# linnanwang/FastGen

Measured on AMD Instinct MI355X. Metric: images/sec at 4-step distilled (DMD2) sampling, higher is better.
Workload: dtype fp32 (tensors, accumulate) with split-bf16 x3 MFMA conv products; 1 GPU; EDM CIFAR-10 32x32 SongUNet (55.7M params) DMD2 4-step 'sde' sampling, batch=512 per GPU; global_batch=512, sample_steps=4, parallelism=replicas x1 (no data-path collective), graph=True

## Files before the change

### fastgen_amd/_lib.py

```python
import ctypes
import os
from ctypes import POINTER, c_char_p, c_double, c_float, c_int, c_int64, c_size_t, c_uint64, c_void_p

_HERE = os.path.dirname(os.path.abspath(__file__))
LIB_PATH = os.path.join(_HERE, "libfastgen_amd.so")

FG_MAX_LEVELS = 8
FG_DTYPE_F32, FG_DTYPE_BF16, FG_DTYPE_BF16X3 = 0, 1, 2
DTYPE_NAMES = {"fp32": FG_DTYPE_F32, "bf16": FG_DTYPE_BF16, "bf16x3": FG_DTYPE_BF16X3}
FG_SAMPLE_SDE, FG_SAMPLE_ODE = 0, 1
SAMPLE_TYPES = {"sde": FG_SAMPLE_SDE, "ode": FG_SAMPLE_ODE}
FG_LOOP_X0, FG_LOOP_MEANFLOW, FG_LOOP_EULER = 0, 1, 2
LOOP_KINDS = {"x0": FG_LOOP_X0, "meanflow": FG_LOOP_MEANFLOW, "euler": FG_LOOP_EULER}
FG_SCHEDULE_EDM, FG_SCHEDULE_RF = 0, 1
FG_DROP_PRECOND_INPUT, FG_DROP_PRECOND_OUTPUT = 1, 2
FG_BWD_DECODER, FG_BWD_ENCODER, FG_BWD_EMBED = 1, 2, 4
FG_MODEL_SONGUNET, FG_MODEL_DHARIWAL = 0, 1


class fg_edm_config(ctypes.Structure):
    _fields_ = [
        ("img_resolution", c_int), ("img_channels", c_int), ("label_dim", c_int), ("augment_dim", c_int),
        ("model_channels", c_int), ("num_levels", c_int), ("channel_mult", c_int * FG_MAX_LEVELS),
        ("channel_mult_emb", c_int), ("num_blocks", c_int), ("num_attn_resolutions", c_int),
# ... 44 lines not shown
    "fg_edm_destroy": (None, [c_void_p]),
    "fg_edm_num_params": (c_int, [c_void_p]),
    "fg_edm_param_info": (c_int, [c_void_p, c_int, POINTER(c_char_p), POINTER(c_int), POINTER(c_int64)]),
    "fg_edm_bind_param": (c_int, [c_void_p, c_char_p, c_void_p, c_int64]),
    "fg_edm_pack_weights": (c_int, [c_void_p, c_void_p]),
    "fg_edm_workspace_bytes": (c_size_t, [c_void_p, c_int]),
    "fg_edm_forward": (c_int, [c_void_p, c_void_p, c_void_p, c_void_p, c_void_p, c_void_p, c_void_p, c_int, c_void_p,
                               c_size_t, c_void_p]),
    "fg_edm_num_feature_taps": (c_int, [c_void_p]),
    "fg_edm_feature_info": (c_int, [c_void_p, c_int, POINTER(c_char_p), POINTER(c_int), POINTER(c_int)]),
    "fg_edm_forward_features": (c_int, [c_void_p, c_void_p, c_void_p, c_void_p, c_void_p, c_void_p, POINTER(c_void_p), c_int,
                                        c_void_p, c_size_t, c_void_p]),
    "fg_sampler_run": (c_int, [c_void_p, c_void_p, c_void_p, POINTER(c_double), c_int, c_int, c_int, c_void_p, c_uint64,
                               c_void_p, c_int, c_void_p, c_size_t, c_int, c_void_p]),
    "fg_edm_t_list": (c_int, [c_int, POINTER(c_double)]),
    "fg_rf_t_list": (c_int, [c_int, POINTER(c_double)]),
    "fg_edm_profile_begin": (c_int, [c_void_p]),
    "fg_edm_profile_end": (c_int, [c_void_p, POINTER(c_int64), POINTER(c_double), POINTER(c_double)]),
    "fg_edm_num_blocks": (c_int, [c_void_p]),
    "fg_edm_block_info": (c_int, [c_void_p, c_int, POINTER(c_char_p), POINTER(c_int), POINTER(c_int), POINTER(c_int),
                                  POINTER(c_int), POINTER(c_int)]),
    "fg_edm_run_block": (c_int, [c_void_p, c_int, c_void_p, c_int, c_void_p, c_int, c_void_p, c_void_p, c_int, c_void_p,
                                 c_size_t, c_void_p]),
    "fg_op_gn_coeffs": (c_int, [c_void_p, c_int, c_void_p, c_int, c_void_p, c_void_p, c_float, c_void_p, c_int, c_int, c_void_p]),
    "fg_op_adm_conv_pack_bytes": (c_size_t, [c_int, c_int, c_int, c_int]),
    "fg_op_adm_conv_pack": (c_int, [c_int, c_void_p, c_void_p, c_int, c_int, c_int, c_void_p]),
    "fg_op_adm_conv": (c_int, [c_int, c_int, c_void_p, c_int, c_void_p, c_int, c_int, c_int, c_int, c_int, c_void_p, c_int, c_void_p,
                               c_void_p, c_void_p, c_int, c_void_p, c_int, c_void_p]),
    "fg_op_adm_gn_workspace_bytes": (c_size_t, [c_int, c_int, c_int]),
    "fg_op_adm_gn_coeffs": (c_int, [c_void_p, c_int, c_void_p, c_int, c_void_p, c_void_p, c_float, c_void_p, c_int, c_void_p, c_int,
                                    c_int, c_void_p, c_size_t, c_void_p]),
    "fg_op_adm_attention": (c_int, [c_void_p, c_void_p, c_int, c_int, c_int, c_void_p]),
    "fg_op_adm_map_in": (c_int, [c_void_p, c_void_p, c_void_p, c_void_p, c_int, c_void_p, c_int, c_int, c_void_p]),
    "fg_op_latents": (c_int, [c_void_p, c_double, c_void_p, c_int64, c_void_p]),
    "fg_op_forward_process": (c_int, [c_void_p, c_void_p, c_double, c_int, c_void_p, c_int64, c_void_p]),
    "fg_op_x0_to_eps": (c_int, [c_void_p, c_void_p, c_double, c_int, c_void_p, c_int64, c_void_p]),
    "fg_op_conv_wgrad_workspace_bytes": (ctypes.c_size_t, [c_int, c_int, c_int, c_int, c_int]),
    "fg_op_conv_wgrad": (c_int, [c_void_p, c_void_p, c_void_p, c_int, c_int, c_int, c_int, c_int, c_int, c_void_p, ctypes.c_size_t, c_void_p]),
    "fg_op_conv_wgrad_f32": (c_int, [c_void_p, c_void_p, c_void_p, c_int, c_int, c_int, c_int, c_int, c_int, c_void_p, ctypes.c_size_t, c_void_p]),
    "fg_edm_bind_grad": (c_int, [c_void_p, c_char_p, c_void_p, c_int64]),
    "fg_edm_block_backward_workspace_bytes": (c_size_t, [c_void_p, c_int, c_int]),
    "fg_edm_run_block_backward": (c_int, [c_void_p, c_int, c_void_p, c_int, c_void_p, c_int, c_void_p, c_void_p, c_void_p,
                                          c_void_p, c_void_p, c_int, c_void_p, c_size_t, c_void_p]),
    "fg_edm_backward_workspace_bytes": (c_size_t, [c_void_p, c_int]),
    "fg_edm_backward": (c_int, [c_void_p, c_void_p, c_void_p, c_void_p, c_void_p, c_void_p, c_void_p, c_int, c_int, c_void_p,
                                c_size_t, c_void_p]),
# ... 101 lines not shown
```

### fastgen_amd/csrc/conv.h

```cpp
#pragma once
#include <hip/hip_runtime.h>

struct ConvArgs {
    const void* src1;
    const void* src2;
    int C1, C2;
    int Hs, Ws;
    int H, W;
    int B;
    const float2* ab;
    const void* wpack;
    const void* wpack_ws;
    const float* bias;
    const float* temb;
    int temb_stride;
    const void* resid;
    int rshift = 0;
    float scale;
    void* out;
    int Cout;
    float2* stats;
    int dbg;
    void* q_out;
    void* k_out;
// ... 2 lines not shown
    int gate_stride = 0;
    int act = 0;
    int heads = 0, head_dim = 0;
    size_t heads_lo_off = 0;
};

enum { PRO_NONE = 0, PRO_GN = 1, PRO_GN_SILU = 2 };
enum { RES_NONE = 0, RES_DOWN = 1, RES_UP = 2, RES_SUBPIX = 3 };
enum { OUT_NHWC = 0, OUT_QKV = 1, OUT_TOK = 2, OUT_HEADS = 3 };

int launch_conv_fused(int dtype, int ks, int pro, int res, int outmode, const ConvArgs& a, hipStream_t stream);
int conv_stat_slots(int W);
bool conv_ws_supported(int dtype, int ks, int pro, int res, int outmode, const ConvArgs& a);
bool conv_ws_enabled();
int launch_conv_ws(int res, const ConvArgs& a, hipStream_t stream, bool prepare_only, int pro = PRO_GN_SILU);
bool conv_ws_shape_ok(int dtype, int cout, int cin, int res);
int launch_pack_conv_weights_ws(const float* w_oihw, void* wpack_ws, int cout, int cin, hipStream_t stream);
bool conv_x3ws_supported(int ks, int pro, int res, int outmode, const ConvArgs& a);
bool conv_x3ws_shape_ok(int cout, int cin, int res);
int conv_x3ws_stat_slots(int W, int res);
int launch_conv_x3ws(int res, const ConvArgs& a, hipStream_t stream, bool prepare_only, int pro = PRO_GN_SILU);
int launch_pack_conv_weights_x3ws(const float* w_oihw, void* wpack_ws, int cout, int cin, hipStream_t stream);
int launch_pack_conv_weights_x3sub(const float* w_oihw, void* wpack_sub, int cout, int cin, hipStream_t stream);
int conv_subpix_mode();
int conv_launch_stat_slots(int dtype, int ks, int pro, int res, int outmode, const ConvArgs& a);
int launch_conv_ws_debug(const ConvArgs& a, int abl, hipStream_t stream);
int launch_conv_debug(int dtype, const ConvArgs& a, hipStream_t stream);
int conv_prepare_all(int dtype);
size_t conv_pack_elems(int cout, int cin, int ks);
int launch_pack_conv_weights(int dtype, const float* w_oihw, void* wpack, int cout, int cin, int ks, int qkv_perm,
                             hipStream_t stream);
```

### fastgen_amd/csrc/conv.hip

```cpp
#include "common.h"
#include "conv.h"
#include <stdlib.h>
#include <string.h>

#include <type_traits>

namespace {

constexpr int PITCH = 144;
constexpr int NTHR = 256;

template <int KS, int LOGW>
struct Geom {
    static constexpr int W = 1 << LOGW;
    static constexpr int LOGTW = (LOGW == 5) ? 4 : LOGW;
    static constexpr int TW = 1 << LOGTW;
    static constexpr int LOGTH = 3;
    static constexpr int TH = 1 << LOGTH;
    static constexpr int IMGS = 128 / (TH * TW);
    static constexpr int TCOLS = W / TW;
    static constexpr int TPI = (IMGS > 1) ? 1 : (W / TH) * TCOLS;
    static constexpr int PAD = KS / 2;
    static constexpr int HW_ = TW + 2 * PAD;
    static constexpr int HH_ = TH + 2 * PAD;
// ... 558 lines not shown
        case 4: return launch_one<__bf16, 3, PRO_GN_SILU, RES_NONE, 5, OUT_NHWC, 4>(a, stream);
        case 5: return launch_one<__bf16, 3, PRO_GN_SILU, RES_NONE, 5, OUT_NHWC, 5>(a, stream);
        case 6: return launch_one<__bf16, 3, PRO_GN_SILU, RES_NONE, 5, OUT_NHWC, 6>(a, stream);
        case 7: return launch_one<__bf16, 3, PRO_GN_SILU, RES_NONE, 5, OUT_NHWC, 7>(a, stream);
    }
    return (int)hipErrorInvalidValue;
}

int launch_conv_fused(int dtype, int ks, int pro, int res, int outmode, const ConvArgs& a, hipStream_t stream) {
    const int kc = dtype == 1 ? DT<__bf16>::KC : DT<float>::KC;
    if (a.H != a.W || (a.W != 8 && a.W != 16 && a.W != 32)) return (int)hipErrorInvalidValue;
    const bool tok = outmode == OUT_TOK || outmode == OUT_HEADS;
    if ((a.C1 % kc) || (a.C2 % kc) || (a.Cout % (tok ? 64 : 256)) || a.B <= 0) return (int)hipErrorInvalidValue;
    if (outmode == OUT_HEADS && (a.heads <= 0 || (a.head_dim % 4) || a.Cout != 3 * a.heads * a.head_dim || ((a.heads * a.head_dim) % 64) ||
                                 !a.q_out || !a.k_out || !a.vt_out))
        return (int)hipErrorInvalidValue;
    if (res == RES_NONE && (a.Hs != a.H || a.Ws != a.W)) return (int)hipErrorInvalidValue;
    if (res == RES_DOWN && (a.Hs != 2 * a.H || a.Ws != 2 * a.W)) return (int)hipErrorInvalidValue;
    if ((res == RES_UP || res == RES_SUBPIX) && (2 * a.Hs != a.H || 2 * a.Ws != a.W)) return (int)hipErrorInvalidValue;
    if (pro != PRO_NONE && !a.ab) return (int)hipErrorInvalidValue;
    if (outmode == OUT_QKV && (a.Cout != 768 || a.W > 16)) return (int)hipErrorInvalidValue;
    if (conv_ws_enabled() && conv_ws_supported(dtype, ks, pro, res, outmode, a)) return launch_conv_ws(res, a, stream, false, pro);
    if (dtype == 2 && conv_ws_enabled() && conv_x3ws_supported(ks, pro, res, outmode, a)) return launch_conv_x3ws(res, a, stream, false, pro);
    if (res == RES_SUBPIX || a.rshift) return (int)hipErrorInvalidValue;
    return dispatch_t(dtype, ks, pro, res, outmode, a, stream);
}

bool conv_ws_enabled() {
    static const bool on = [] {
        const char* e = getenv("FASTGEN_AMD_CONV_WS");
        return !(e && e[0] == '0');
    }();
    return on;
}

int conv_subpix_mode() {
    static const int mode = [] {
        const char* e = getenv("FASTGEN_AMD_CONV_SUBPIX");
        if (e && e[0] == '0') return 0;
        return (e && !strcmp(e, "skip")) ? 1 : 2;
    }();
    return mode;
}

int conv_launch_stat_slots(int dtype, int ks, int pro, int res, int outmode, const ConvArgs& a) {
    if (dtype == 2 && conv_ws_enabled() && conv_x3ws_supported(ks, pro, res, outmode, a)) return conv_x3ws_stat_slots(a.W, res);
// ... 16 lines not shown
                rc = dispatch_t(dtype, 3, PRO_GN_SILU, res, OUT_NHWC, a, nullptr);
            if (!rc) rc = dispatch_t(dtype, 1, PRO_NONE, res, OUT_NHWC, a, nullptr);
        }
        if (!rc) rc = dispatch_t(dtype, 3, PRO_NONE, RES_NONE, OUT_NHWC, a, nullptr);
        if (!rc && a.W <= 16) rc = dispatch_t(dtype, 1, PRO_GN, RES_NONE, OUT_QKV, a, nullptr);
        if (!rc && a.W == 16) rc = dispatch_t(dtype, 1, PRO_NONE, RES_NONE, OUT_TOK, a, nullptr);
        if (!rc && a.W == 16) rc = dispatch_t(dtype, 1, PRO_NONE, RES_NONE, OUT_HEADS, a, nullptr);
    }
    g_prepare_only = false;
    if (!rc && dtype == 2) {
        ConvArgs w{};
        for (int res : {RES_NONE, RES_UP})
            for (int ww : {32, 16, 8}) {
                if (ww == 8 && res != RES_NONE) continue;
                w.W = w.H = ww;
                if (!rc) rc = launch_conv_x3ws(res, w, nullptr, true, PRO_GN_SILU);
                if (!rc && res == RES_NONE) rc = launch_conv_x3ws(res, w, nullptr, true, PRO_NONE);
            }
        for (int ws_ : {16, 8}) {
            w.Ws = w.Hs = ws_;
            w.W = w.H = 2 * ws_;
            if (!rc) rc = launch_conv_x3ws(RES_SUBPIX, w, nullptr, true, PRO_GN_SILU);
        }
    }
    if (!rc && dtype == 1) {
        ConvArgs w{};
        for (int res : {RES_NONE, RES_UP}) {
            w.W = w.H = 32;
            if (!rc) rc = launch_conv_ws(res, w, nullptr, true);
            if (res == RES_NONE) {
                w.C1 = -128;
                if (!rc) rc = launch_conv_ws(res, w, nullptr, true);
                w.C1 = 0;
            }
            w.W = w.H = 16;
            if (!rc) rc = launch_conv_ws(res, w, nullptr, true);
        }
    }
    return rc;
}

size_t conv_pack_elems(int cout, int cin, int ks) { return (size_t)cout * cin * ks * ks; }

int launch_pack_conv_weights(int dtype, const float* w, void* out, int cout, int cin, int ks, int qkv_perm,
                             hipStream_t stream) {
    const size_t total = conv_pack_elems(cout, cin, ks);
// ... 10 lines not shown
```

### fastgen_amd/csrc/engine.hip

```cpp
#include <hip/hip_runtime.h>

#include <cmath>
#include <cstdarg>
#include <cstdio>
#include <cstdlib>
#include <cstring>
#include <string>
#include <map>
#include <vector>

#include "../../include/fastgen_amd.h"
#include "common.h"
#include "adm.h"
#include "edm2.h"
#include "conv.h"
#include "misc.h"

namespace {

thread_local std::string g_err;

int fail(int code, const char* fmt, ...) {
    char buf[512];
    va_list ap;
// ... 12 lines not shown

struct Param {
    std::string name;
    int ndim = 0;
    int64_t shape[4] = {1, 1, 1, 1};
    int64_t numel = 0;
    const float* ptr = nullptr;
    float* grad = nullptr;
};

enum Kind { K_STEM, K_BLOCK, K_AUX_NORM, K_AUX_CONV };

struct Block {
    std::string key;
    Kind kind = K_BLOCK;
    int cin = 0, cout = 0, res_in = 0, res_out = 0;
    bool up = false, down = false, attn = false, has_skip = false, is_dec = false;
    int skip_c = 0;
    int temb_off = 0;
    int norm0_w = -1, norm0_b = -1, conv0_w = -1, conv0_b = -1, aff_w = -1, aff_b = -1, norm1_w = -1, norm1_b = -1,
        conv1_w = -1, conv1_b = -1, skip_w = -1, skip_b = -1, norm2_w = -1, norm2_b = -1, qkv_w = -1, qkv_b = -1,
        proj_w = -1, proj_b = -1, w = -1, b = -1;
    void *p_conv0 = nullptr, *p_conv1 = nullptr, *p_skip = nullptr, *p_qkv = nullptr, *p_proj = nullptr;
    void *p_conv0_ws = nullptr, *p_conv1_ws = nullptr;
    void* p_conv0_sub = nullptr;
    int tap = -1;
    float* qkv_bias = nullptr;
    void* p_aux = nullptr;
    void* p_stem = nullptr;
};

struct Arena {
    char* base = nullptr;
    size_t off = 0, cap = 0;
    bool dry = false;
    void* take(size_t bytes) {
        off = (off + 255) & ~(size_t)255;
        void* p = dry ? nullptr : base + off;
        off += bytes;
        return p;
    }
    template <typename T>
    T* get(size_t n) {
        return reinterpret_cast<T*>(take(n * sizeof(T)));
    }
};
// ... 623 lines not shown
        HIP_TRY(launch_gn_finalize(x1.st, c1, x1.slots, c2 ? x2.st : nullptr, c2, c2 ? x2.slots : 0, gamma, beta, kBlockEps, ab, B, hw, s, mr));
    else
        HIP_TRY(launch_gn_coeffs(dtype, x1.p, c1, c2 ? x2.p : nullptr, c2, gamma, beta, kBlockEps, ab, B, hw, s, mr));
    return FG_OK;
}

void use_stash(Workspace& w, const BlockStash& st) {
    w.h.p = st.h;
    w.ab0 = st.ab0, w.ab1 = st.ab1, w.mr0 = st.mr0, w.mr1 = st.mr1;
    w.a1d = st.a1d;
    w.drop.block = st.index;
    if (st.xattn) {
        w.xattn.p = st.xattn;
        w.ab2 = st.ab2, w.mr2 = st.mr2;
        w.q = st.q, w.k = st.k, w.vt = st.vt, w.aout = st.aout;
    }
}
int block_index(const fg_edm* h, const Block* b) {
    for (size_t i = 0; i < h->blocks.size(); ++i)
        if (h->blocks[i] == b) return (int)i;
    return -1;
}

int run_block(fg_edm* h, const Block& b, const Act& x1, int c1, const Act& x2, int c2, const float* temb, Act& out, int B,
              Workspace& w, hipStream_t s) {
    if (c1 + c2 != b.cin) return fail(FG_EINVAL, "%s: got %d+%d input channels, expected %d", b.key.c_str(), c1, c2, b.cin);
    const int hw_in = b.res_in * b.res_in, hw = b.res_out * b.res_out;
    const int res_mode = b.down ? RES_DOWN : (b.up ? RES_UP : RES_NONE);
    const int slots = conv_stat_slots(b.res_out);
    int rc;
    if ((rc = norm_coeffs(h->dtype, x1, c1, x2, c2, h->P(b.norm0_w), h->P(b.norm0_b), w.ab0, B, hw_in, s, w.mr0))) return rc;
    ConvArgs a{};
    a.src1 = x1.p; a.src2 = c2 ? x2.p : nullptr; a.C1 = c1; a.C2 = c2;
    a.Hs = a.Ws = b.res_in; a.H = a.W = b.res_out; a.B = B;
    a.ab = w.ab0; a.wpack = b.p_conv0; a.wpack_ws = b.p_conv0_ws; a.bias = h->P(b.conv0_b);
    a.temb = temb + b.temb_off; a.temb_stride = h->temb_total;
    a.resid = nullptr; a.scale = 1.0f; a.out = w.h.p; a.Cout = b.cout; a.stats = w.h.st;
    const bool x3_up = b.up && w.infer && !w.a1d && h->cmode == FG_DTYPE_BF16X3 && conv_ws_enabled();
    bool sub0 = false;
    if (x3_up && conv_subpix_mode() == 2 && b.p_conv0_sub) {
        ConvArgs p = a;
        p.wpack_ws = b.p_conv0_sub;
        sub0 = conv_x3ws_supported(3, PRO_GN_SILU, RES_SUBPIX, OUT_NHWC, p);
    }
    if (sub0) {
        a.wpack_ws = b.p_conv0_sub;
// ... 22 lines not shown
        }
        ConvArgs k{};
        k.src1 = x1.p; k.src2 = c2 ? x2.p : nullptr; k.C1 = c1; k.C2 = c2;
        k.Hs = k.Ws = b.res_in; k.H = k.W = low ? b.res_in : b.res_out; k.B = B;
        k.wpack = b.p_skip; k.bias = h->P(b.skip_b); k.scale = 1.0f; k.out = w.sbuf; k.Cout = b.cout;
        HIP_TRY(conv_launch(h, 1, PRO_NONE, low ? RES_NONE : res_mode, OUT_NHWC, k, s));
        resid = w.sbuf;
        d.rshift = low ? 1 : 0;
    }
    HIP_TRY(launch_gn_finalize(w.h.st, b.cout, w.h.slots, nullptr, 0, 0, h->P(b.norm1_w), h->P(b.norm1_b), kBlockEps, w.ab1, B, hw, s, w.mr1));
    Act& x_mid = b.attn ? w.xattn : out;
    d.resid = resid; d.out = x_mid.p; d.stats = x_mid.st;
    if (w.a1d) {
        HIP_TRY(launch_gn_act(h->dtype, 0, w.h.p, b.cout, nullptr, 0, w.ab1, w.a1d, B, b.res_out, 0, s, w.drop));
        d.src1 = w.a1d; d.ab = nullptr;
        x_mid.slots = conv_launch_stat_slots(h->cmode, 3, PRO_NONE, RES_NONE, OUT_NHWC, d);
        HIP_TRY(conv_launch(h, 3, PRO_NONE, RES_NONE, OUT_NHWC, d, s));
    } else {
        x_mid.slots = conv_launch_stat_slots(h->cmode, 3, PRO_GN_SILU, RES_NONE, OUT_NHWC, d);
        HIP_TRY(conv_launch(h, 3, PRO_GN_SILU, RES_NONE, OUT_NHWC, d, s));
    }
    if (b.attn) {
        HIP_TRY(launch_gn_finalize(x_mid.st, b.cout, x_mid.slots, nullptr, 0, 0, h->P(b.norm2_w), h->P(b.norm2_b), kBlockEps, w.ab2, B, hw, s, w.mr2));
        ConvArgs q{};
        q.src1 = x_mid.p; q.C1 = b.cout; q.Hs = q.Ws = q.H = q.W = b.res_out; q.B = B;
        q.ab = w.ab2; q.wpack = b.p_qkv; q.bias = b.qkv_bias; q.scale = 1.0f; q.Cout = 3 * b.cout;
        q.q_out = w.q; q.k_out = w.k; q.vt_out = w.vt;
        HIP_TRY(conv_launch(h, 1, PRO_GN, RES_NONE, OUT_QKV, q, s));
        HIP_TRY(launch_attention(h->cmode, w.q, w.k, w.vt, w.aout, B, hw, s));
        ConvArgs p{};
        p.src1 = w.aout; p.C1 = b.cout; p.Hs = p.Ws = p.H = p.W = b.res_out; p.B = B;
        p.wpack = b.p_proj; p.bias = h->P(b.proj_b); p.resid = x_mid.p; p.scale = kSkipScale; p.out = out.p; p.Cout = b.cout;
        p.stats = out.st;
        HIP_TRY(conv_launch(h, 1, PRO_NONE, RES_NONE, OUT_NHWC, p, s));
        out.slots = slots;
    }
    return FG_OK;
}

int run_mapping(fg_edm* h, const float* labels, int B, Workspace& w, hipStream_t s) {
    const fg_edm_config& c = h->cfg;
    HIP_TRY(launch_mapping_in(w.coef + B, w.coef + 4 * (size_t)B, h->freqs, labels, c.label_dim,
                              h->P(h->find("model.map_label.weight")), h->P(h->find("model.map_label.bias")), w.emb0, B,
                              h->cond_ch, h->noise_ch, s, h->augment, h->augment ? h->P(h->find("model.map_augment.weight")) : nullptr, c.augment_dim));
    HIP_TRY(launch_linear(w.emb0, h->P(h->find("model.map_layer0.weight")), h->P(h->find("model.map_layer0.bias")), w.emb1,
                          B, h->cond_ch, h->emb_ch, 1, s));
    HIP_TRY(launch_linear(w.emb1, h->P(h->find("model.map_layer1.weight")), h->P(h->find("model.map_layer1.bias")), w.emb, B,
                          h->emb_ch, h->emb_ch, 1, s));
    HIP_TRY(launch_linear(w.emb, h->aff_w, h->aff_b, w.temb, B, h->emb_ch, h->temb_total, 0, s));
    return FG_OK;
}

int run_forward(fg_edm* h, const float* x_t, const double* t, int t_stride, const double* r, int r_stride,
                const float* labels, float* out, int B, Workspace& w, hipStream_t s, float* const* feats = nullptr,
                bool early = false, TrainStash* ts = nullptr) {
    if (h->adm) return adm_forward(h, x_t, t, t_stride, labels, out, B, w, s);
// ... 68 lines not shown
}

int ensure_device_state(fg_edm* h) {
    if (h->device_ready) return FG_OK;
    int rc;
    const size_t tsz = h->dtype ? 2 : 4;
    for (Block* b : h->blocks) {
        if ((rc = h->alloc(&b->p_conv0, conv_pack_elems(b->cout, b->cin, 3) * tsz))) return rc;
        if ((rc = h->alloc(&b->p_conv1, conv_pack_elems(b->cout, b->cout, 3) * tsz))) return rc;
        const bool x3 = h->cmode == FG_DTYPE_BF16X3;
        if ((x3 ? conv_x3ws_shape_ok(b->cout, b->cin, b->res_out) : conv_ws_shape_ok(h->cmode, b->cout, b->cin, b->res_out)) && !b->down &&
            (rc = h->alloc(&b->p_conv0_ws, conv_pack_elems(b->cout, b->cin, 3) * tsz)))
            return rc;
        if ((x3 ? conv_x3ws_shape_ok(b->cout, b->cout, b->res_out) : conv_ws_shape_ok(h->cmode, b->cout, b->cout, b->res_out)) &&
            (rc = h->alloc(&b->p_conv1_ws, conv_pack_elems(b->cout, b->cout, 3) * tsz)))
            return rc;
        if (x3 && b->up && conv_x3ws_shape_ok(b->cout, b->cin, b->res_in) && (rc = h->alloc(&b->p_conv0_sub, conv_pack_elems(b->cout, b->cin, 4) * 4)))
            return rc;
        if (b->has_skip && (rc = h->alloc(&b->p_skip, conv_pack_elems(b->cout, b->cin, 1) * tsz))) return rc;
        if (b->attn) {
            if ((rc = h->alloc(&b->p_qkv, conv_pack_elems(3 * b->cout, b->cout, 1) * tsz))) return rc;
            if ((rc = h->alloc(&b->p_proj, conv_pack_elems(b->cout, b->cout, 1) * tsz))) return rc;
            if ((rc = h->alloc((void**)&b->qkv_bias, sizeof(float) * 3 * b->cout))) return rc;
        }
    }
    for (Block& b : h->enc)
        if (b.kind == K_STEM && stem_supported(b.res_out, b.cin, b.cout))
            if ((rc = h->alloc(&b.p_stem, stem_pack_elems() * tsz))) return rc;
    for (Block& b : h->dec)
        if (b.kind == K_AUX_CONV && aux_head_supported(h->cmode, b.res_out, b.cin, b.cout))
            if ((rc = h->alloc(&b.p_aux, aux_pack_elems(b.cin) * tsz))) return rc;
    if ((rc = h->alloc((void**)&h->aff_w, sizeof(float) * (size_t)h->temb_total * h->emb_ch))) return rc;
    if ((rc = h->alloc((void**)&h->aff_b, sizeof(float) * (size_t)h->temb_total))) return rc;
    const int half = h->noise_ch / 2;
    std::vector<float> fr(half);
    for (int j = 0; j < half; ++j) fr[j] = powf(1.0f / 10000.0f, (float)j / (float)(half - 1));
    if ((rc = h->alloc((void**)&h->freqs, sizeof(float) * half))) return rc;
    HIP_TRY(hipMemcpy(h->freqs, fr.data(), sizeof(float) * half, hipMemcpyHostToDevice));
    if (conv_prepare_all(h->cmode) != 0) return fail(FG_EHIP, "hipFuncSetAttribute(dynamic LDS) failed");
    if (launch_attention(h->cmode, nullptr, nullptr, nullptr, nullptr, 1, 256, nullptr) != 0) return fail(FG_EHIP, "attention prepare failed");
    h->device_ready = true;
    return FG_OK;
}

#include "engine_adm.inc"

// ... 80 lines not shown
        ++h->pack_epoch;
        if ((rc = adm_pack_weights(h, s))) return rc;
        h->sampler.graph.drop();
        h->packed = true;
        return FG_OK;
    }
    if ((rc = ensure_device_state(h)) || (rc = h->check_bound(unused))) return rc;
    ++h->pack_epoch;
    for (Block* b : h->blocks) {
        HIP_TRY(launch_pack_conv_weights(h->cmode, h->P(b->conv0_w), b->p_conv0, b->cout, b->cin, 3, 0, s));
        HIP_TRY(launch_pack_conv_weights(h->cmode, h->P(b->conv1_w), b->p_conv1, b->cout, b->cout, 3, 0, s));
        if (h->cmode == FG_DTYPE_BF16X3) {
            if (b->p_conv0_ws) HIP_TRY(launch_pack_conv_weights_x3ws(h->P(b->conv0_w), b->p_conv0_ws, b->cout, b->cin, s));
            if (b->p_conv0_sub) HIP_TRY(launch_pack_conv_weights_x3sub(h->P(b->conv0_w), b->p_conv0_sub, b->cout, b->cin, s));
            if (b->p_conv1_ws) HIP_TRY(launch_pack_conv_weights_x3ws(h->P(b->conv1_w), b->p_conv1_ws, b->cout, b->cout, s));
        } else {
            if (b->p_conv0_ws) HIP_TRY(launch_pack_conv_weights_ws(h->P(b->conv0_w), b->p_conv0_ws, b->cout, b->cin, s));
            if (b->p_conv1_ws) HIP_TRY(launch_pack_conv_weights_ws(h->P(b->conv1_w), b->p_conv1_ws, b->cout, b->cout, s));
        }
        if (b->has_skip) HIP_TRY(launch_pack_conv_weights(h->cmode, h->P(b->skip_w), b->p_skip, b->cout, b->cin, 1, 0, s));
        if (b->attn) {
            HIP_TRY(launch_pack_conv_weights(h->cmode, h->P(b->qkv_w), b->p_qkv, 3 * b->cout, b->cout, 1, 1, s));
            HIP_TRY(launch_pack_conv_weights(h->cmode, h->P(b->proj_w), b->p_proj, b->cout, b->cout, 1, 0, s));
            for (int plane = 0; plane < 3; ++plane)
                HIP_TRY(hipMemcpy2DAsync(b->qkv_bias + plane * b->cout, sizeof(float), h->P(b->qkv_b) + plane,
                                         3 * sizeof(float), sizeof(float), b->cout, hipMemcpyDeviceToDevice, s));
        }
        HIP_TRY(hipMemcpyAsync(h->aff_w + (size_t)b->temb_off * h->emb_ch, h->P(b->aff_w),
                               sizeof(float) * (size_t)b->cout * h->emb_ch, hipMemcpyDeviceToDevice, s));
        HIP_TRY(hipMemcpyAsync(h->aff_b + b->temb_off, h->P(b->aff_b), sizeof(float) * b->cout, hipMemcpyDeviceToDevice, s));
    }
    for (Block& b : h->enc)
        if (b.kind == K_STEM && b.p_stem) HIP_TRY(launch_pack_stem_weights(h->dtype, h->P(b.w), b.p_stem, b.cin, s));
    for (Block& b : h->dec)
        if (b.kind == K_AUX_CONV && b.p_aux) HIP_TRY(launch_pack_aux_weights(h->cmode, h->P(b.w), b.p_aux, b.cin, b.cout, s));
    h->sampler.graph.drop();
    h->packed = true;
    return FG_OK;
}

size_t fg_edm_workspace_bytes(const fg_edm* h, int batch) {
    if (!h || batch <= 0) return 0;
    Arena A;
    A.dry = true;
    Workspace w;
    return plan_workspace(h, batch, A, w);
// ... 142 lines not shown
    HIP_TRY(hipMalloc(&wp, (size_t)256 * cin * ks * ks * 4));
    {
        const size_t blk = 4u << 20;
        std::vector<uint16_t> hb(blk / 2);
        uint32_t st = 0x12345u;
        for (auto& v : hb) {
            st = st * 1664525u + 1013904223u;
            v = (uint16_t)(((st >> 16) & 0x8000u) | ((0x78u + ((st >> 12) & 7u)) << 7) | ((st >> 20) & 0x7fu));
        }
        auto fill = [&](void* dst, size_t bytes) -> int {
            for (size_t o = 0; o < bytes; o += blk)
                HIP_TRY(hipMemcpy((char*)dst + o, hb.data(), std::min(blk, bytes - o), hipMemcpyHostToDevice));
            return FG_OK;
        };
        int rc;
        if ((rc = fill(x, npix * cin * 4)) || (rc = fill(resid, npix * 256 * 4)) || (rc = fill(ab, (size_t)batch * cin * 8)) ||
            (rc = fill(wp, (size_t)256 * cin * ks * ks * (dtype == 1 ? 2 : 4))))
            return rc;
    }
    HIP_TRY(hipMemset(bias, 0, 256 * 4));
    if (conv_prepare_all(dtype) != 0) return fail(FG_EHIP, "prepare failed");
    ConvArgs a{};
    a.src1 = x; a.C1 = cin; a.Hs = a.Ws = a.H = a.W = res; a.B = batch;
    a.ab = ab; a.wpack = wp; a.wpack_ws = wp; a.bias = bias; a.resid = with_resid ? resid : nullptr; a.scale = 1.f; a.out = out; a.Cout = 256;
    a.dbg = dbg;
    hipEvent_t e0, e1;
    HIP_TRY(hipEventCreate(&e0));
    HIP_TRY(hipEventCreate(&e1));
    auto run = [&]() { return dbg >= 64 ? launch_conv_ws_debug(a, dbg - 64, nullptr) : dbg < 0 ? launch_conv_fused(dtype, ks, ks == 3 ? PRO_GN_SILU : PRO_NONE, RES_NONE, OUT_NHWC, a, nullptr) : launch_conv_debug(dtype, a, nullptr); };
    for (int i = 0; i < 3; ++i) HIP_TRY(run());
    HIP_TRY(hipEventRecord(e0, nullptr));
    for (int i = 0; i < iters; ++i) HIP_TRY(run());
    HIP_TRY(hipEventRecord(e1, nullptr));
    HIP_TRY(hipEventSynchronize(e1));
    float ms = 0.f;
    HIP_TRY(hipEventElapsedTime(&ms, e0, e1));
    if (ms_out) *ms_out = ms / iters;
    (void)hipEventDestroy(e0); (void)hipEventDestroy(e1);
    (void)hipFree(x); (void)hipFree(out); (void)hipFree(resid); (void)hipFree(bias); (void)hipFree(ab); (void)hipFree(wp);
    return FG_OK;
}

int fg_edm_num_blocks(const fg_edm* h) {
    if (h && h->adm) return adm_num_blocks(h);
    return h ? (int)h->blocks.size() : 0;
}

// ... 15 lines not shown
                     int batch, void* workspace, size_t workspace_bytes, void* stream) {
    if (!h || !x1 || !emb || !out) return fail(FG_EINVAL, "null argument");
    if (h->adm) return adm_run_block(h, index, x1, c1, x2, c2, emb, out, batch, workspace, workspace_bytes, (hipStream_t)stream);
    if (!h->packed) return fail(FG_ENOTREADY, "weights are not packed (call fg_edm_pack_weights)");
    if (index < 0 || index >= (int)h->blocks.size()) return fail(FG_EINVAL, "block index out of range");
    Workspace w;
    int rc0 = setup_ws(plan_workspace, h, batch, workspace, workspace_bytes, w);
    if (rc0) return rc0;
    hipStream_t s = (hipStream_t)stream;
    HIP_TRY(launch_linear(emb, h->aff_w, h->aff_b, w.temb, batch, h->emb_ch, h->temb_total, 0, s));
    const Block& b = *h->blocks[index];
    const size_t npix_in = (size_t)batch * b.res_in * b.res_in, npix_out = (size_t)batch * b.res_out * b.res_out;
    Act a1, a2;
    HIP_TRY(launch_to_act(h->dtype, x1, w.cvt1, (int64_t)npix_in * c1, s));
    a1.p = w.cvt1;
    if (c2) {
        HIP_TRY(launch_to_act(h->dtype, x2, w.cvt2, (int64_t)npix_in * c2, s));
        a2.p = w.cvt2;
    }
    w.infer = true;
    int rc = run_block(h, b, a1, c1, a2, c2, w.temb, w.xa, batch, w, s);
    if (rc) return rc;
    HIP_TRY(launch_from_act(h->dtype, w.xa.p, out, (int64_t)npix_out * b.cout, s));
    return FG_OK;
}

#include "engine_train.inc"
#include "engine_dit.inc"
#include "engine_wan.inc"
#include "engine_sampler.inc"
#include "engine_edm2.inc"

int fg_op_gn_coeffs(const float* x1, int c1, const float* x2, int c2, const float* gamma, const float* beta, float eps,
                    float* ab_out, int batch, int hw, void* stream) {
    if (!x1 || !gamma || !beta || !ab_out) return fail(FG_EINVAL, "null argument");
    HIP_TRY(launch_gn_coeffs(0, x1, c1, c2 ? x2 : nullptr, c2, gamma, beta, eps, (float2*)ab_out, batch, hw, (hipStream_t)stream));
    return FG_OK;
}

size_t fg_op_adm_conv_pack_bytes(int mode, int cout, int cin, int ks) {
    if ((mode != FG_DTYPE_BF16 && mode != FG_DTYPE_BF16X3) || (ks != 1 && ks != 3) || cout <= 0 || cin <= 0 || cin % 32) return 0;
    return adm_conv_pack_elems(mode, cout, cin, ks) * sizeof(__bf16);
}
int fg_op_adm_conv_pack(int mode, const float* w_oihw, void* packed, int cout, int cin, int ks, void* stream) {
    if (!fg_op_adm_conv_pack_bytes(mode, cout, cin, ks))
        return fail(FG_EINVAL, "fg_op_adm_conv_pack: mode %d (1 bf16, 2 bf16x3), ks %d (1, 3), cout %d > 0, cin %d (multiple of 32)", mode,
// ... 270 lines not shown
```

### include/fastgen_amd.h

```cpp
#ifndef FASTGEN_AMD_H
#define FASTGEN_AMD_H

#include <stddef.h>
#include <stdint.h>

#ifdef __cplusplus
extern "C" {
#endif

#define FG_API __attribute__((visibility("default")))

#define FG_OK 0
#define FG_EINVAL 1
#define FG_ENOTREADY 2
#define FG_EHIP 3
#define FG_ENOMEM 4

#define FG_DTYPE_F32 0
#define FG_DTYPE_BF16 1
#define FG_DTYPE_BF16X3 2

#define FG_SAMPLE_SDE 0
#define FG_SAMPLE_ODE 1

// ... 55 lines not shown

FG_API int fg_edm_num_feature_taps(const fg_edm* h);
FG_API int fg_edm_feature_info(const fg_edm* h, int index, const char** key, int* channels, int* resolution);
FG_API int fg_edm_forward_features(fg_edm* h, const float* x_t, const double* t, const double* r, const float* class_labels,
                            float* out, float* const* features, int batch, void* workspace, size_t workspace_bytes,
                            void* stream);

FG_API int fg_sampler_run(fg_edm* h, const float* noise, const float* class_labels, const double* t_list, int steps,
                   int sample_type, int loop_kind, const float* eps, uint64_t seed, float* out, int batch,
                   void* workspace, size_t workspace_bytes, int use_graph, void* stream);

FG_API int fg_edm_t_list(int sample_steps, double* out_host);
FG_API int fg_rf_t_list(int sample_steps, double* out_host);

FG_API int fg_edm_profile_begin(fg_edm* h);
FG_API int fg_edm_profile_end(fg_edm* h, int64_t* launches, double* total_ms, double* total_flops);


FG_API int fg_edm_num_blocks(const fg_edm* h);
FG_API int fg_edm_block_info(const fg_edm* h, int index, const char** key, int* cin, int* cout, int* res_in, int* res_out,
                      int* has_attention);
FG_API int fg_edm_run_block(fg_edm* h, int index, const float* x1, int c1, const float* x2, int c2, const float* emb,
                     float* out, int batch, void* workspace, size_t workspace_bytes, void* stream);

FG_API int fg_op_gn_coeffs(const float* x1, int c1, const float* x2, int c2, const float* gamma, const float* beta,
                    float eps, float* ab_out, int batch, int hw, void* stream);

FG_API size_t fg_op_adm_conv_pack_bytes(int mode, int cout, int cin, int ks);
FG_API int fg_op_adm_conv_pack(int mode, const float* w_oihw, void* packed, int cout, int cin, int ks, void* stream);
FG_API int fg_op_adm_conv(int mode, int ks, const float* src1, int c1, const float* src2, int c2, int batch, int hs, int h,
                          int res_mode, const float* ab, int silu, const void* packed, const float* bias, const float* resid,
                          int resid_mode, float* out, int cout, void* stream);
FG_API size_t fg_op_adm_gn_workspace_bytes(int batch, int hw, int c);
FG_API int fg_op_adm_gn_coeffs(const float* x1, int c1, const float* x2, int c2, const float* gamma, const float* beta, float eps,
                               const float* temb, int temb_stride, float* ab_out, int batch, int hw, void* workspace,
                               size_t workspace_bytes, void* stream);
FG_API int fg_op_adm_attention(const float* qkv, float* out, int batch, int t, int heads, void* stream);
FG_API int fg_op_adm_map_in(const float* c_noise, const float* freqs, const float* aug, const float* wa, int aug_dim, float* out,
                            int batch, int n, void* stream);

FG_API int fg_op_latents(const float* noise, double t_init, float* out, int64_t total, void* stream);
FG_API int fg_op_forward_process(const float* x0, const float* eps, double t, int schedule, float* out, int64_t total,
                          void* stream);
FG_API int fg_op_x0_to_eps(const float* xt, const float* x0, double t, int schedule, float* out, int64_t total, void* stream);
FG_API size_t fg_op_conv_wgrad_workspace_bytes(int batch, int res, int cin, int cout, int ks);
FG_API int fg_op_conv_wgrad(const void* act, const void* dy, float* dw, int batch, int res, int cin, int cout, int ks,
// ... 199 lines not shown
```

Baseline: 2829 img/s.

## Add dedicated split-bf16x3 1x1 conv kernel for attention QKV projection

Adds a specialised 1x1 convolution kernel for 256-channel attention blocks under split-bf16x3. It stages a 128-pixel tile of GroupNorm-applied inputs as hi/lo bf16 planes in LDS, streams pre-packed hi/lo weights through a register ring with buffer loads, and writes Q, K and transposed V directly. It is enabled by default for the QKV conv at inference. The output projection path is also covered but only runs when an environment variable is set to 'all'. The intent is to replace the generic conv dispatch for these GEMM-like 1x1 convs with a better-scheduled MFMA pipeline, at the cost of extra packed weight memory and a new code path to validate.

```diff
diff --git a/fastgen_amd/_lib.py b/fastgen_amd/_lib.py
--- a/fastgen_amd/_lib.py
+++ b/fastgen_amd/_lib.py
@@ -90,6 +90,7 @@
                                   POINTER(c_int), POINTER(c_int)]),
     "fg_edm_run_block": (c_int, [c_void_p, c_int, c_void_p, c_int, c_void_p, c_int, c_void_p, c_void_p, c_int, c_void_p,
                                  c_size_t, c_void_p]),
+    "fg_edm_block_qkv": (c_int, [c_void_p, c_int, c_void_p, c_void_p, c_void_p, c_void_p, c_int, c_void_p, c_size_t, c_void_p]),
     "fg_op_gn_coeffs": (c_int, [c_void_p, c_int, c_void_p, c_int, c_void_p, c_void_p, c_float, c_void_p, c_int, c_int, c_void_p]),
     "fg_op_adm_conv_pack_bytes": (c_size_t, [c_int, c_int, c_int, c_int]),
     "fg_op_adm_conv_pack": (c_int, [c_int, c_void_p, c_void_p, c_int, c_int, c_int, c_void_p]),
diff --git a/fastgen_amd/csrc/conv.h b/fastgen_amd/csrc/conv.h
--- a/fastgen_amd/csrc/conv.h
+++ b/fastgen_amd/csrc/conv.h
@@ -48,6 +48,11 @@
 int launch_conv_x3ws(int res, const ConvArgs& a, hipStream_t stream, bool prepare_only, int pro = PRO_GN_SILU);
 int launch_pack_conv_weights_x3ws(const float* w_oihw, void* wpack_ws, int cout, int cin, hipStream_t stream);
 int launch_pack_conv_weights_x3sub(const float* w_oihw, void* wpack_sub, int cout, int cin, hipStream_t stream);
+bool conv1_x3_supported(int pro, int res, int outmode, const ConvArgs& a);
+bool conv1_x3_shape_ok(int cout, int cin, int res);
+int launch_conv1_x3(int pro, int outmode, const ConvArgs& a, hipStream_t stream, bool prepare_only);
+int launch_pack_conv_weights_x3c1(const float* w_oihw, void* wpack, int cout, int cin, int qkv_perm, hipStream_t stream);
+int conv1_x3_mode();
 int conv_subpix_mode();
 int conv_launch_stat_slots(int dtype, int ks, int pro, int res, int outmode, const ConvArgs& a);
 int launch_conv_ws_debug(const ConvArgs& a, int abl, hipStream_t stream);
diff --git a/fastgen_amd/csrc/conv.hip b/fastgen_amd/csrc/conv.hip
--- a/fastgen_amd/csrc/conv.hip
+++ b/fastgen_amd/csrc/conv.hip
@@ -604,6 +604,8 @@
     if (outmode == OUT_QKV && (a.Cout != 768 || a.W > 16)) return (int)hipErrorInvalidValue;
     if (conv_ws_enabled() && conv_ws_supported(dtype, ks, pro, res, outmode, a)) return launch_conv_ws(res, a, stream, false, pro);
     if (dtype == 2 && conv_ws_enabled() && conv_x3ws_supported(ks, pro, res, outmode, a)) return launch_conv_x3ws(res, a, stream, false, pro);
+    if (dtype == 2 && ks == 1 && a.wpack_ws && conv1_x3_mode() && conv1_x3_supported(pro, res, outmode, a))
+        return launch_conv1_x3(pro, outmode, a, stream, false);
     if (res == RES_SUBPIX || a.rshift) return (int)hipErrorInvalidValue;
     return dispatch_t(dtype, ks, pro, res, outmode, a, stream);
 }
@@ -666,6 +668,8 @@
             w.W = w.H = 2 * ws_;
             if (!rc) rc = launch_conv_x3ws(RES_SUBPIX, w, nullptr, true, PRO_GN_SILU);
         }
+        if (!rc) rc = launch_conv1_x3(PRO_GN, OUT_QKV, w, nullptr, true);
+        if (!rc) rc = launch_conv1_x3(PRO_NONE, OUT_NHWC, w, nullptr, true);
     }
     if (!rc && dtype == 1) {
         ConvArgs w{};
diff --git a/fastgen_amd/csrc/conv1_x3.hip b/fastgen_amd/csrc/conv1_x3.hip
--- /dev/null
+++ b/fastgen_amd/csrc/conv1_x3.hip
@@ -0,0 +1,274 @@
+#include "common.h"
+#include "conv.h"
+#include <stdlib.h>
+#include <string.h>
+
+namespace {
+
+constexpr int C1_NTHR = 512;
+constexpr int C1_CIN = 256;
+constexpr int C1_PLANE = 2048;
+constexpr int C1_LO = 32 * C1_PLANE;
+constexpr int C1_LDS = 2 * C1_LO;
+constexpr int C1_STEPB = 2048;
+constexpr int C1_GRPB = 8 * C1_STEPB;
+constexpr int C1_RN = 4;
+
+struct C1Frag {
+    bf16x8 hi, lo;
+};
+
+__device__ __forceinline__ C1Frag c1_load_w(const __amdgpu_buffer_rsrc_t wrs, int wvoff, int byte_off) {
+    C1Frag f;
+    f.hi = __builtin_bit_cast(bf16x8, __builtin_amdgcn_raw_buffer_load_b128(wrs, wvoff, byte_off, 0));
+    f.lo = __builtin_bit_cast(bf16x8, __builtin_amdgcn_raw_buffer_load_b128(wrs, wvoff, byte_off + 1024, 0));
+    return f;
+}
+
+template <bool TR>
+__device__ __forceinline__ void conv1_x3_pass(const char* xlane, const __amdgpu_buffer_rsrc_t wrs, const int wvoff, const int wcur,
+                                              const int wnxt, C1Frag (&wq)[C1_RN][2], f32x4 (&acc)[8][2]) {
+    constexpr int NQ = 32;
+    auto read_x = [&](int q, C1Frag (&xf)[2]) {
+        const int off = (q >> 2) * (4 * C1_PLANE) + 2 * (q & 3) * 256;
+#pragma unroll
+        for (int m = 0; m < 2; ++m) {
+            xf[m].hi = *reinterpret_cast<const bf16x8*>(xlane + off + m * 256);
+            xf[m].lo = *reinterpret_cast<const bf16x8*>(xlane + off + m * 256 + C1_LO);
+        }
+    };
+    auto mma = [&](f32x4 c, bf16x8 w, bf16x8 x) -> f32x4 {
+        return TR ? __builtin_amdgcn_mfma_f32_16x16x32_bf16(x, w, c, 0, 0, 0) : __builtin_amdgcn_mfma_f32_16x16x32_bf16(w, x, c, 0, 0, 0);
+    };
+    auto mma12 = [&](int q, const C1Frag (&xf)[2]) {
+        const int step = q >> 2, m0 = 2 * (q & 3);
+        const C1Frag(&wf)[2] = wq[step % C1_RN];
+#pragma unroll
+        for (int m = 0; m < 2; ++m)
+#pragma unroll
+            for (int nt = 0; nt < 2; ++nt) acc[m0 + m][nt] = mma(acc[m0 + m][nt], wf[nt].hi, xf[m].lo);
+#pragma unroll
+        for (int m = 0; m < 2; ++m)
+#pragma unroll
+            for (int nt = 0; nt < 2; ++nt) acc[m0 + m][nt] = mma(acc[m0 + m][nt], wf[nt].lo, xf[m].hi);
+#pragma unroll
+        for (int m = 0; m < 2; ++m)
+#pragma unroll
+            for (int nt = 0; nt < 2; ++nt) acc[m0 + m][nt] = mma(acc[m0 + m][nt], wf[nt].hi, xf[m].hi);
+        if ((q & 3) != 3) return;
+        const int pn = (step + C1_RN < 8) ? wcur + (step + C1_RN) * C1_STEPB : wnxt + (step + C1_RN - 8) * C1_STEPB;
+#pragma unroll
+        for (int nt = 0; nt < 2; ++nt) wq[step % C1_RN][nt] = c1_load_w(wrs, wvoff, pn + nt * C1_GRPB);
+    };
+#pragma unroll
+    for (int m = 0; m < 8; ++m)
+#pragma unroll
+        for (int nt = 0; nt < 2; ++nt) acc[m][nt] = f32x4{0.f, 0.f, 0.f, 0.f};
+    C1Frag x0[2], x1[2];
+    read_x(0, x0);
+#pragma unroll
+    for (int q = 0; q < NQ; q += 2) {
+        read_x(q + 1, x1);
+        __builtin_amdgcn_sched_barrier(0);
+        mma12(q, x0);
+        __builtin_amdgcn_sched_barrier(0);
+        if (q + 2 < NQ) read_x(q + 2, x0);
+        __builtin_amdgcn_sched_barrier(0);
+        mma12(q + 1, x1);
+        __builtin_amdgcn_sched_barrier(0);
+    }
+}
+
+template <int PRO, int OUTMODE>
+__global__ __launch_bounds__(C1_NTHR) void conv1_x3_kernel(const ConvArgs a) {
+    extern __shared__ __attribute__((aligned(16))) char smem[];
+    const int tid = threadIdx.x;
+    const int lane = tid & 63;
+    const int wave = __builtin_amdgcn_readfirstlane(tid >> 6);
+    const int col = lane & 15, g4 = lane >> 4;
+    const int tile = (int)gridDim.x - 1 - (int)blockIdx.x;
+    const int HW = a.H * a.W;
+    const int n = tile * 128 / HW;
+    const int p0 = tile * 128 - n * HW;
+    const size_t gp0 = (size_t)tile * 128;
+
+    const __amdgpu_buffer_rsrc_t wrs = __builtin_amdgcn_make_buffer_rsrc(
+        const_cast<__bf16*>(reinterpret_cast<const __bf16*>(a.wpack_ws)) + (size_t)wave * (2 * C1_GRPB / 2), 0, 0x7fffffff, 0x00020000);
+    const int wvoff = lane * 16;
+    constexpr int PASSB = 16 * C1_GRPB;
+    constexpr int NPASS = OUTMODE == OUT_QKV ? 3 : 1;
+    C1Frag wq[C1_RN][2];
+#pragma unroll
+    for (int j = 0; j < C1_RN; ++j)
+#pragma unroll
+        for (int nt = 0; nt < 2; ++nt) wq[j][nt] = c1_load_w(wrs, wvoff, nt * C1_GRPB + j * C1_STEPB);
+
+    const int cw = wave * 32 + 4 * g4;
+    float* const out = reinterpret_cast<float*>(a.out);
+    const size_t ob = (gp0 + col) * 256 + cw;
+    const bool has_resid = OUTMODE == OUT_NHWC && __builtin_amdgcn_readfirstlane(a.resid != nullptr);
+    f32x4 rr[8][2];
+    if (OUTMODE == OUT_NHWC && has_resid) {
+        const float* resid = reinterpret_cast<const float*>(a.resid);
+#pragma unroll
+        for (int m = 0; m < 8; ++m)
+#pragma unroll
+            for (int nt = 0; nt < 2; ++nt) rr[m][nt] = *reinterpret_cast<const f32x4*>(resid + ob + m * (16 * 256) + nt * 16);
+    }
+
+    {
+        const float* src = reinterpret_cast<const float*>(a.src1) + (gp0 + wave * 16 + col) * C1_CIN + g4 * 8;
+        const float2* abn = a.ab + (size_t)n * C1_CIN + g4 * 8;
+        char* const dst = smem + g4 * C1_PLANE + (wave * 16 + col) * 16;
+        f32x4 raw[8][2];
+#pragma unroll
+        for (int s = 0; s < 8; ++s) {
+            raw[s][0] = *reinterpret_cast<const f32x4*>(src + s * 32);
+            raw[s][1] = *reinterpret_cast<const f32x4*>(src + s * 32 + 4);
+        }
+#pragma unroll
+        for (int s = 0; s < 8; ++s) {
+            float v[8];
+#pragma unroll
+            for (int j = 0; j < 8; ++j) v[j] = raw[s][j >> 2][j & 3];
+            if (PRO != PRO_NONE) {
+#pragma unroll
+                for (int j = 0; j < 8; j += 2) {
+                    const f32x4 c = *reinterpret_cast<const f32x4*>(abn + s * 32 + j);
+                    v[j] = fmaf(v[j], c[0], c[1]);
+                    v[j + 1] = fmaf(v[j + 1], c[2], c[3]);
+                }
+            }
+            bf16x8 hi, lo;
+            split8(v, hi, lo);
+            *reinterpret_cast<bf16x8*>(dst + s * (4 * C1_PLANE)) = hi;
+            *reinterpret_cast<bf16x8*>(dst + s * (4 * C1_PLANE) + C1_LO) = lo;
+        }
+    }
+    __syncthreads();
+
+    const char* const xlane = smem + g4 * C1_PLANE + col * 16;
+    f32x4 acc[8][2];
+#pragma unroll 1
+    for (int p = 0; p < (OUTMODE == OUT_QKV ? 2 : 1); ++p) {
+        conv1_x3_pass<false>(xlane, wrs, wvoff, p * PASSB, (p + 1 < NPASS) ? (p + 1) * PASSB : p * PASSB, wq, acc);
+        if (OUTMODE == OUT_QKV) {
+            float* const plane = reinterpret_cast<float*>(p == 0 ? a.q_out : a.k_out);
+#pragma unroll
+            for (int nt = 0; nt < 2; ++nt) {
+                f32x4 bias4 = {0.f, 0.f, 0.f, 0.f};
+                if (a.bias) bias4 = *reinterpret_cast<const f32x4*>(a.bias + p * 256 + cw + nt * 16);
+#pragma unroll
+                for (int m = 0; m < 8; ++m) *reinterpret_cast<f32x4*>(plane + ob + m * (16 * 256) + nt * 16) = acc[m][nt] + bias4;
+            }
+        } else {
+#pragma unroll
+            for (int nt = 0; nt < 2; ++nt) {
+                f32x4 bias4 = {0.f, 0.f, 0.f, 0.f};
+                if (a.bias) bias4 = *reinterpret_cast<const f32x4*>(a.bias + cw + nt * 16);
+                float ssum = 0.f, ssq = 0.f;
+#pragma unroll
+                for (int m = 0; m < 8; ++m) {
+                    f32x4 v = acc[m][nt] + bias4;
+                    if (has_resid) v += rr[m][nt];
+                    v *= a.scale;
+                    *reinterpret_cast<f32x4*>(out + ob + m * (16 * 256) + nt * 16) = v;
+                    ssum += (v[0] + v[1]) + (v[2] + v[3]);
+                    ssq += (v[0] * v[0] + v[1] * v[1]) + (v[2] * v[2] + v[3] * v[3]);
+                }
+#pragma unroll
+                for (int sh = 1; sh < 16; sh <<= 1) {
+                    ssum += __shfl_xor(ssum, sh);
+                    ssq += __shfl_xor(ssq, sh);
+                }
+                if (a.stats && col == 0) a.stats[(size_t)tile * 64 + ((cw + nt * 16) >> 2)] = make_float2(ssum, ssq);
+            }
+        }
+    }
+    if (OUTMODE == OUT_QKV) {
+        conv1_x3_pass<true>(xlane, wrs, wvoff, 2 * PASSB, 2 * PASSB, wq, acc);
+        float* const vt = reinterpret_cast<float*>(a.vt_out);
+#pragma unroll
+        for (int nt = 0; nt < 2; ++nt) {
+            const int ch = wave * 32 + nt * 16 + col;
+            const float bias = a.bias ? a.bias[512 + ch] : 0.f;
+            float* const row = vt + ((size_t)n * 256 + ch) * HW + p0 + 4 * g4;
+#pragma unroll
+            for (int m = 0; m < 8; ++m) *reinterpret_cast<f32x4*>(row + m * 16) = acc[m][nt] + bias;
+        }
+    }
+}
+
+__global__ void pack_conv_weights_x3c1_kernel(const float* __restrict__ w, __bf16* __restrict__ out, int cout, int cin, int qkv_perm) {
+    const size_t total = (size_t)cout * cin;
+    const int nstep = cin / 32;
+    for (size_t idx = (size_t)blockIdx.x * blockDim.x + threadIdx.x; idx < total; idx += (size_t)gridDim.x * blockDim.x) {
+        size_t t = idx;
+        const int j = t % 8; t /= 8;
+        const int lane = t % 64; t /= 64;
+        const int step = t % nstep; t /= nstep;
+        const int n16 = (int)t;
+        int co = n16 * 16 + (lane & 15);
+        if (qkv_perm) {
+            const int C = cout / 3;
+            co = (co % C) * 3 + co / C;
+        }
+        const int ci = step * 32 + 8 * (lane >> 4) + j;
+        const float v = w[(size_t)co * cin + ci];
+        const __bf16 hi = (__bf16)v;
+        const size_t o = (idx / 512) * 1024 + (idx % 512);
+        out[o] = hi;
+        out[o + 512] = (__bf16)(v - (float)hi);
+    }
+}
+
+template <int PRO, int OUTMODE>
+int launch_c1_one(const ConvArgs& a, hipStream_t stream, bool prepare_only) {
+    auto kern = conv1_x3_kernel<PRO, OUTMODE>;
+    const int dev = fg_device_slot();
+    if (dev < 0) return (int)hipErrorInvalidDevice;
+    static bool attr_done[16] = {};
+    if (!attr_done[dev]) {
+        hipError_t e = hipFuncSetAttribute(reinterpret_cast<const void*>(kern), hipFuncAttributeMaxDynamicSharedMemorySize, C1_LDS);
+        if (e != hipSuccess) return (int)e;
+        attr_done[dev] = true;
+    }
+    if (prepare_only) return 0;
+    const int ntiles = (int)((size_t)a.B * a.H * a.W / 128);
+    hipLaunchKernelGGL(kern, dim3(ntiles), dim3(C1_NTHR), C1_LDS, stream, a);
+    return (int)hipGetLastError();
+}
+
+}
+
+int conv1_x3_mode() {
+    static const int mode = [] {
+        const char* e = getenv("FASTGEN_AMD_CONV1_X3");
+        if (e && e[0] == '0') return 0;
+        return (e && !strcmp(e, "all")) ? 2 : 1;
+    }();
+    return mode;
+}
+
+bool conv1_x3_shape_ok(int cout, int cin, int res) { return cin == C1_CIN && (cout == 256 || cout == 768) && res > 0 && (res * res) % 128 == 0; }
+
+bool conv1_x3_supported(int pro, int res, int outmode, const ConvArgs& a) {
+    if (res != RES_NONE || a.C1 != C1_CIN || a.C2 != 0 || !a.src1 || !a.wpack_ws || a.temb || a.rshift || a.B <= 0) return false;
+    if (a.H != a.W || a.Hs != a.H || a.Ws != a.W || !conv1_x3_shape_ok(a.Cout, C1_CIN, a.W)) return false;
+    if ((size_t)a.B * a.H * a.W / 128 > 0x7fffffu) return false;
+    if (pro != PRO_NONE && (pro != PRO_GN || !a.ab)) return false;
+    if (outmode == OUT_QKV) return a.Cout == 768 && pro == PRO_GN && a.scale == 1.0f && a.q_out && a.k_out && a.vt_out;
+    return outmode == OUT_NHWC && a.Cout == 256 && pro == PRO_NONE && a.out && a.H * a.W / 128 == conv_stat_slots(a.W);
+}
+
+int launch_conv1_x3(int pro, int outmode, const ConvArgs& a, hipStream_t stream, bool prepare_only) {
+    if (outmode == OUT_QKV) return launch_c1_one<PRO_GN, OUT_QKV>(a, stream, prepare_only);
+    return launch_c1_one<PRO_NONE, OUT_NHWC>(a, stream, prepare_only);
+}
+
+int launch_pack_conv_weights_x3c1(const float* w_oihw, void* wpack, int cout, int cin, int qkv_perm, hipStream_t stream) {
+    const size_t total = (size_t)cout * cin;
+    const int grid = (int)((total + 255) / 256 < 4096 ? (total + 255) / 256 : 4096);
+    hipLaunchKernelGGL(pack_conv_weights_x3c1_kernel, dim3(grid), dim3(256), 0, stream, w_oihw, (__bf16*)wpack, cout, cin, qkv_perm);
+    return (int)hipGetLastError();
+}
diff --git a/fastgen_amd/csrc/engine.hip b/fastgen_amd/csrc/engine.hip
--- a/fastgen_amd/csrc/engine.hip
+++ b/fastgen_amd/csrc/engine.hip
@@ -58,6 +58,7 @@
         conv1_w = -1, conv1_b = -1, skip_w = -1, skip_b = -1, norm2_w = -1, norm2_b = -1, qkv_w = -1, qkv_b = -1,
         proj_w = -1, proj_b = -1, w = -1, b = -1;
     void *p_conv0 = nullptr, *p_conv1 = nullptr, *p_skip = nullptr, *p_qkv = nullptr, *p_proj = nullptr;
+    void *p_qkv_c1 = nullptr, *p_proj_c1 = nullptr;
     void *p_conv0_ws = nullptr, *p_conv1_ws = nullptr;
     void* p_conv0_sub = nullptr;
     int tap = -1;
@@ -727,6 +728,16 @@
     return -1;
 }
 
+int launch_block_qkv(fg_edm* h, const Block& b, const void* x, int B, Workspace& w, bool c1, hipStream_t s) {
+    ConvArgs q{};
+    q.src1 = x; q.C1 = b.cout; q.Hs = q.Ws = q.H = q.W = b.res_out; q.B = B;
+    q.ab = w.ab2; q.wpack = b.p_qkv; q.bias = b.qkv_bias; q.scale = 1.0f; q.Cout = 3 * b.cout;
+    q.q_out = w.q; q.k_out = w.k; q.vt_out = w.vt;
+    if (c1) q.wpack_ws = b.p_qkv_c1;
+    HIP_TRY(conv_launch(h, 1, PRO_GN, RES_NONE, OUT_QKV, q, s));
+    return FG_OK;
+}
+
 int run_block(fg_edm* h, const Block& b, const Act& x1, int c1, const Act& x2, int c2, const float* temb, Act& out, int B,
               Workspace& w, hipStream_t s) {
     if (c1 + c2 != b.cin) return fail(FG_EINVAL, "%s: got %d+%d input channels, expected %d", b.key.c_str(), c1, c2, b.cin);
@@ -795,16 +806,14 @@
     }
     if (b.attn) {
         HIP_TRY(launch_gn_finalize(x_mid.st, b.cout, x_mid.slots, nullptr, 0, 0, h->P(b.norm2_w), h->P(b.norm2_b), kBlockEps, w.ab2, B, hw, s, w.mr2));
-        ConvArgs q{};
-        q.src1 = x_mid.p; q.C1 = b.cout; q.Hs = q.Ws = q.H = q.W = b.res_out; q.B = B;
-        q.ab = w.ab2; q.wpack = b.p_qkv; q.bias = b.qkv_bias; q.scale = 1.0f; q.Cout = 3 * b.cout;
-        q.q_out = w.q; q.k_out = w.k; q.vt_out = w.vt;
-        HIP_TRY(conv_launch(h, 1, PRO_GN, RES_NONE, OUT_QKV, q, s));
+        const bool c1 = w.infer && !w.a1d && h->cmode == FG_DTYPE_BF16X3;
+        HIP_TRY(launch_block_qkv(h, b, x_mid.p, B, w, c1, s));
         HIP_TRY(launch_attention(h->cmode, w.q, w.k, w.vt, w.aout, B, hw, s));
         ConvArgs p{};
         p.src1 = w.aout; p.C1 = b.cout; p.Hs = p.Ws = p.H = p.W = b.res_out; p.B = B;
         p.wpack = b.p_proj; p.bias = h->P(b.proj_b); p.resid = x_mid.p; p.scale = kSkipScale; p.out = out.p; p.Cout = b.cout;
         p.stats = out.st;
+        if (c1 && conv1_x3_mode() == 2) p.wpack_ws = b.p_proj_c1;
         HIP_TRY(conv_launch(h, 1, PRO_NONE, RES_NONE, OUT_NHWC, p, s));
         out.slots = slots;
     }
@@ -919,6 +928,10 @@
             if ((rc = h->alloc(&b->p_qkv, conv_pack_elems(3 * b->cout, b->cout, 1) * tsz))) return rc;
             if ((rc = h->alloc(&b->p_proj, conv_pack_elems(b->cout, b->cout, 1) * tsz))) return rc;
             if ((rc = h->alloc((void**)&b->qkv_bias, sizeof(float) * 3 * b->cout))) return rc;
+            if (x3 && conv1_x3_shape_ok(3 * b->cout, b->cout, b->res_out)) {
+                if ((rc = h->alloc(&b->p_qkv_c1, conv_pack_elems(3 * b->cout, b->cout, 1) * 4))) return rc;
+                if ((rc = h->alloc(&b->p_proj_c1, conv_pack_elems(b->cout, b->cout, 1) * 4))) return rc;
+            }
         }
     }
     for (Block& b : h->enc)
@@ -1045,6 +1058,8 @@
         if (b->attn) {
             HIP_TRY(launch_pack_conv_weights(h->cmode, h->P(b->qkv_w), b->p_qkv, 3 * b->cout, b->cout, 1, 1, s));
             HIP_TRY(launch_pack_conv_weights(h->cmode, h->P(b->proj_w), b->p_proj, b->cout, b->cout, 1, 0, s));
+            if (b->p_qkv_c1) HIP_TRY(launch_pack_conv_weights_x3c1(h->P(b->qkv_w), b->p_qkv_c1, 3 * b->cout, b->cout, 1, s));
+            if (b->p_proj_c1) HIP_TRY(launch_pack_conv_weights_x3c1(h->P(b->proj_w), b->p_proj_c1, b->cout, b->cout, 0, s));
             for (int plane = 0; plane < 3; ++plane)
                 HIP_TRY(hipMemcpy2DAsync(b->qkv_bias + plane * b->cout, sizeof(float), h->P(b->qkv_b) + plane,
                                          3 * sizeof(float), sizeof(float), b->cout, hipMemcpyDeviceToDevice, s));
@@ -1233,7 +1248,7 @@
     if (conv_prepare_all(dtype) != 0) return fail(FG_EHIP, "prepare failed");
     ConvArgs a{};
     a.src1 = x; a.C1 = cin; a.Hs = a.Ws = a.H = a.W = res; a.B = batch;
-    a.ab = ab; a.wpack = wp; a.wpack_ws = wp; a.bias = bias; a.resid = with_resid ? resid : nullptr; a.scale = 1.f; a.out = out; a.Cout = 256;
+    a.ab = ab; a.wpack = wp; a.wpack_ws = ks == 3 ? wp : nullptr; a.bias = bias; a.resid = with_resid ? resid : nullptr; a.scale = 1.f; a.out = out; a.Cout = 256;
     a.dbg = dbg;
     hipEvent_t e0, e1;
     HIP_TRY(hipEventCreate(&e0));
@@ -1295,6 +1310,29 @@
     int rc = run_block(h, b, a1, c1, a2, c2, w.temb, w.xa, batch, w, s);
     if (rc) return rc;
     HIP_TRY(launch_from_act(h->dtype, w.xa.p, out, (int64_t)npix_out * b.cout, s));
+    return FG_OK;
+}
+
+int fg_edm_block_qkv(fg_edm* h, int index, const float* x, float* q, float* k, float* vt, int batch, void* workspace,
+                     size_t workspace_bytes, void* stream) {
+    if (!h || !x || !q || !k || !vt) return fail(FG_EINVAL, "null argument");
+    if (h->adm) return adm_refuse(h, "fg_edm_block_qkv");
+    if (!h->packed) return fail(FG_ENOTREADY, "weights are not packed (call fg_edm_pack_weights)");
+    if (index < 0 || index >= (int)h->blocks.size() || !h->blocks[index]->attn) return fail(FG_EINVAL, "not an attention block");
+    Workspace w;
+    int rc0 = setup_ws(plan_workspace, h, batch, workspace, workspace_bytes, w);
+    if (rc0) return rc0;
+    hipStream_t s = (hipStream_t)stream;
+    const Block& b = *h->blocks[index];
+    const int hw = b.res_out * b.res_out;
+    const int64_t n = (int64_t)batch * hw * b.cout;
+    HIP_TRY(launch_to_act(h->dtype, x, w.xattn.p, n, s));
+    HIP_TRY(launch_gn_coeffs(h->dtype, w.xattn.p, b.cout, nullptr, 0, h->P(b.norm2_w), h->P(b.norm2_b), kBlockEps, w.ab2, batch, hw, s, nullptr));
+    int rc = launch_block_qkv(h, b, w.xattn.p, batch, w, h->cmode == FG_DTYPE_BF16X3, s);
+    if (rc) return rc;
+    HIP_TRY(launch_from_act(h->dtype, w.q, q, n, s));
+    HIP_TRY(launch_from_act(h->dtype, w.k, k, n, s));
+    HIP_TRY(launch_from_act(h->dtype, w.vt, vt, n, s));
     return FG_OK;
 }
 
diff --git a/include/fastgen_amd.h b/include/fastgen_amd.h
--- a/include/fastgen_amd.h
+++ b/include/fastgen_amd.h
@@ -101,6 +101,8 @@
                       int* has_attention);
 FG_API int fg_edm_run_block(fg_edm* h, int index, const float* x1, int c1, const float* x2, int c2, const float* emb,
                      float* out, int batch, void* workspace, size_t workspace_bytes, void* stream);
+FG_API int fg_edm_block_qkv(fg_edm* h, int index, const float* x, float* q, float* k, float* vt, int batch, void* workspace,
+                     size_t workspace_bytes, void* stream);
 
 FG_API int fg_op_gn_coeffs(const float* x1, int c1, const float* x2, int c2, const float* gamma, const float* beta,
                     float eps, float* ab_out, int batch, int hw, void* stream);
```

Measured after the change: 2841 img/s, median of 6. No clear change (+0.4%).
